# BBischof/ESRecsys

Hardware: AMD Instinct MI355X
Metric: training pairs/sec (higher is better)
Workload: dtype f32; 1 GPU; inbatch: V=1000000 x D=128 fp32 tables, B=8192, sparse Adagrad; score_precision=auto -> f16x2, ids=uniform, parallelism=single

## Files before the change

### esrecsys_amd/csrc/esr_inbatch2h.hip

```cpp
#include "esr_inbatch_mfma.h"
#include "esr_segment.h"
#include <atomic>
#include <type_traits>
#include <time.h>

namespace esr {

typedef _Float16 f16x8 __attribute__((ext_vector_type(8)));
typedef _Float16 f16x2 __attribute__((ext_vector_type(2)));

constexpr int kHLseOff = 2 * kPlaneBytes;
constexpr int kHBufBytes = kHLseOff + 4 * 256;
constexpr float kHOptHead = 4.0f;
constexpr float kHOverflow = 60000.0f;
constexpr int kHBufs = 3;
constexpr float kHPexp = 14.0f;
constexpr float kHBoundSafe = 14.0f;
constexpr int kHScaleWords = 8;

#define H_MFMA(a, b, c) __builtin_amdgcn_mfma_f32_32x32x16_f16((a), (b), (c), 0, 0, 0)
#define H_SB() __builtin_amdgcn_sched_barrier(0)
#define H_DMA_BARRIER()                                 \
  {                                                     \
    asm volatile("s_waitcnt vmcnt(0)" ::: "memory");    \
// ... 195 lines not shown
  for (int o = 32; o > 0; o >>= 1) {
    mq = fmaxf(mq, __shfl_xor(mq, o, 64));
    mc = fmaxf(mc, __shfl_xor(mc, o, 64));
  }
  if ((t & 63) == 0) { red[t >> 6] = mq; red[4 + (t >> 6)] = mc; }
  __syncthreads();
  mq = fmaxf(fmaxf(red[0], red[1]), fmaxf(red[2], red[3]));
  mc = fmaxf(fmaxf(red[4], red[5]), fmaxf(red[6], red[7]));
  const int eq = scale_exp(mq), ec = scale_exp(mc);
  if (blockIdx.x == 0 && blockIdx.y == 0 && t == 0) {
    sc[0] = ldexpf(1.f, -(eq + ec));
    sc[1] = ldexpf(1.f, -ec);
    sc[2] = ldexpf(1.f, -(eq + (int)kHPexp));
    sc[3] = ldexpf(1.f, eq);
    sc[4] = ldexpf(1.f, ec);
  }
  const RowSrc X = blockIdx.y ? X1 : X0;
  _Float16* R = blockIdx.y ? R1 : R0;
  const float mul = ldexpf(1.f, blockIdx.y ? ec : eq);
  const int chunk = blockIdx.x;
  const int row = t >> 3, d0 = (t & 7) * 16;
  const int64_t grow = (int64_t)chunk * 32 + row;
  float v[16];
#pragma unroll
  for (int q = 0; q < 4; ++q) {
    const float4 f = rowsrc_load4(X, grow, d0 + 4 * q);
    v[4 * q] = f.x; v[4 * q + 1] = f.y; v[4 * q + 2] = f.z; v[4 * q + 3] = f.w;
  }
  {
    float ss = 0.f;
#pragma unroll
    for (int e = 0; e < 16; ++e) ss = fmaf(v[e], v[e], ss);
    ss += __shfl_xor(ss, 1, 64);
    ss += __shfl_xor(ss, 2, 64);
    ss += __shfl_xor(ss, 4, 64);
    ss = fmaxf(ss, __shfl_xor(ss, 8, 64));
    ss = fmaxf(ss, __shfl_xor(ss, 16, 64));
    ss = fmaxf(ss, __shfl_xor(ss, 32, 64));
    if ((t & 63) == 0) nrm[((int64_t)blockIdx.y * gridDim.x + chunk) * 4 + (t >> 6)] = ss;
  }
  f16x8 p[2][2];
#pragma unroll
  for (int e = 0; e < 16; ++e) {
    const float xs = v[e] * mul;
    const _Float16 a = (_Float16)xs;
    const _Float16 b = (_Float16)(xs - (float)a);
    p[0][e >> 3][e & 7] = a;
    p[1][e >> 3][e & 7] = b;
  }
#pragma unroll
  for (int pl = 0; pl < 2; ++pl) {
    f16x8* dst = reinterpret_cast<f16x8*>(R + ((int64_t)pl * B + grow) * k3D + d0);
    dst[0] = p[pl][0];
    dst[1] = p[pl][1];
  }
}

constexpr unsigned long long kPollTicks = 300000000ull;
__device__ __forceinline__ unsigned amax_code(float amax) {
  if (!(amax > 0.f)) return 0u;
  if (!(amax < INFINITY)) return 255u;
  int x;
  frexpf(amax, &x);
  return (unsigned)min(max(x + 127, 1), 254);
}
__device__ __forceinline__ int scale_exp_code(unsigned code) {
  if (code == 0u || code == 255u) return 0;
  const int e = 14 - ((int)code - 127);
  return e < -100 ? -100 : (e > 100 ? 100 : e);
}

__global__ __launch_bounds__(256) void prepsplit2h_kernel(RowSrc X0, RowSrc X1, int64_t B, _Float16* __restrict__ R0,
                                                         _Float16* __restrict__ R1,
                                                         unsigned long long* __restrict__ ent,
                                                         unsigned long long token, float* __restrict__ diag,
                                                         float* __restrict__ nrm, float* __restrict__ sc,
                                                         unsigned long long* __restrict__ loss_acc,
                                                         int* __restrict__ flags, int nflags,
                                                         float* __restrict__ copy0, float* __restrict__ copy1,
                                                         unsigned* __restrict__ czero, int two_level) {
  __shared__ float red[8];
  __shared__ unsigned cred[8];
  const int t = threadIdx.x, chunk = blockIdx.x, nchunks = gridDim.x;
  if (chunk == 0 && t <= kLossWords) {
    loss_acc[t * 16] = 0ull;
    if (t == 0) loss_acc[8] = 0ull;
  }
  if (chunk == 1 || nchunks == 1)
    for (int i = t; i < nflags; i += 256) flags[i] = 0;
  if (czero && chunk == 0 && t < 16) czero[t] = 0u;
  const int row = t >> 3, d0 = (t & 7) * 16;
  const int64_t grow = (int64_t)chunk * 32 + row;
  float vq[16], vc[16];
  {
    const int64_t rq = X0.idx ? (int64_t)X0.idx[grow] : grow;
    const int64_t rc = X1.idx ? (int64_t)X1.idx[grow] : grow;
    RowSrc Y0 = X0, Y1 = X1;
    Y0.idx = nullptr; Y1.idx = nullptr;
#pragma unroll
    for (int q = 0; q < 4; ++q) {
      const float4 f = rowsrc_load4(Y0, rq, d0 + 4 * q);
      const float4 g = rowsrc_load4(Y1, rc, d0 + 4 * q);
      vq[4 * q] = f.x; vq[4 * q + 1] = f.y; vq[4 * q + 2] = f.z; vq[4 * q + 3] = f.w;
      vc[4 * q] = g.x; vc[4 * q + 1] = g.y; vc[4 * q + 2] = g.z; vc[4 * q + 3] = g.w;
      if (copy0 && d0 + 4 * q < X0.ld) *reinterpret_cast<float4*>(copy0 + grow * X0.ld + d0 + 4 * q) = f;
      if (copy1 && d0 + 4 * q < X1.ld) *reinterpret_cast<float4*>(copy1 + grow * X1.ld + d0 + 4 * q) = g;
    }
  }
  float mq = 0.f, mc = 0.f, dot = 0.f, ssq = 0.f, ssc = 0.f;
#pragma unroll
  for (int e = 0; e < 16; ++e) {
    mq = fmaxf(mq, fabsf(vq[e]));
    mc = fmaxf(mc, fabsf(vc[e]));
    dot = fmaf(vq[e], vc[e], dot);
    ssq = fmaf(vq[e], vq[e], ssq);
    ssc = fmaf(vc[e], vc[e], ssc);
  }
  dot += __shfl_xor(dot, 1, 64); dot += __shfl_xor(dot, 2, 64); dot += __shfl_xor(dot, 4, 64);
  ssq += __shfl_xor(ssq, 1, 64); ssq += __shfl_xor(ssq, 2, 64); ssq += __shfl_xor(ssq, 4, 64);
  ssc += __shfl_xor(ssc, 1, 64); ssc += __shfl_xor(ssc, 2, 64); ssc += __shfl_xor(ssc, 4, 64);
  if ((t & 7) == 0) diag[grow] = dot;
#pragma unroll
  for (int o = 8; o < 64; o <<= 1) {
    ssq = fmaxf(ssq, __shfl_xor(ssq, o, 64));
    ssc = fmaxf(ssc, __shfl_xor(ssc, o, 64));
  }
  if ((t & 63) == 0) {
    nrm[((int64_t)0 * nchunks + chunk) * 4 + (t >> 6)] = ssq;
    nrm[((int64_t)1 * nchunks + chunk) * 4 + (t >> 6)] = ssc;
  }
#pragma unroll
  for (int o = 32; o > 0; o >>= 1) {
    mq = fmaxf(mq, __shfl_xor(mq, o, 64));
    mc = fmaxf(mc, __shfl_xor(mc, o, 64));
  }
  if ((t & 63) == 0) { red[t >> 6] = mq; red[4 + (t >> 6)] = mc; }
  __syncthreads();
  if (t == 0) {
    mq = fmaxf(fmaxf(red[0], red[1]), fmaxf(red[2], red[3]));
    mc = fmaxf(fmaxf(red[4], red[5]), fmaxf(red[6], red[7]));
    __hip_atomic_store(&ent[chunk], (token << 16) | (unsigned long long)(amax_code(mq) << 8 | amax_code(mc)),
                       __ATOMIC_RELAXED, __HIP_MEMORY_SCOPE_AGENT);
  }
  unsigned cq = 0u, cc = 0u;
  bool timed_out = false;
  const unsigned long long t_start = __builtin_amdgcn_s_memrealtime();
  const bool gatherer = chunk == 0 || !two_level;
  for (int i = gatherer ? t : (t == 0 ? nchunks : nchunks + 1); i < (gatherer ? nchunks : nchunks + 1); i += 256) {
    unsigned long long v;
    while (((v = __hip_atomic_load(&ent[i], __ATOMIC_RELAXED, __HIP_MEMORY_SCOPE_AGENT)) >> 16) != token) {
      if (__builtin_amdgcn_s_memrealtime() - t_start > kPollTicks) { timed_out = true; break; }
      __builtin_amdgcn_s_sleep(4);
    }
    cq = max(cq, (unsigned)(v >> 8) & 255u);
    cc = max(cc, (unsigned)v & 255u);
  }
  if (timed_out) atomicOr(reinterpret_cast<unsigned*>(loss_acc + 8), 1u);
#pragma unroll
  for (int o = 32; o > 0; o >>= 1) {
    cq = max(cq, (unsigned)__shfl_xor((int)cq, o, 64));
    cc = max(cc, (unsigned)__shfl_xor((int)cc, o, 64));
  }
  if ((t & 63) == 0) { cred[t >> 6] = cq; cred[4 + (t >> 6)] = cc; }
  __syncthreads();
  cq = max(max(cred[0], cred[1]), max(cred[2], cred[3]));
  cc = max(max(cred[4], cred[5]), max(cred[6], cred[7]));
  if (two_level && chunk == 0 && t == 0)
    __hip_atomic_store(&ent[nchunks], (token << 16) | (unsigned long long)(cq << 8 | cc), __ATOMIC_RELAXED,
                       __HIP_MEMORY_SCOPE_AGENT);
  const int eq = scale_exp_code(cq), ec = scale_exp_code(cc);
  if (chunk == 0 && t == 0) {
    sc[0] = ldexpf(1.f, -(eq + ec));
    sc[1] = ldexpf(1.f, -ec);
    sc[2] = ldexpf(1.f, -(eq + (int)kHPexp));
    sc[3] = ldexpf(1.f, eq);
    sc[4] = ldexpf(1.f, ec);
  }
#pragma unroll
  for (int m = 0; m < 2; ++m) {
    const float mul = ldexpf(1.f, m ? ec : eq);
    _Float16* R = m ? R1 : R0;
    f16x8 p[2][2];
#pragma unroll
    for (int e = 0; e < 16; ++e) {
      const float xs = (m ? vc[e] : vq[e]) * mul;
      const _Float16 a = (_Float16)xs;
      const _Float16 b = (_Float16)(xs - (float)a);
      p[0][e >> 3][e & 7] = a;
      p[1][e >> 3][e & 7] = b;
    }
#pragma unroll
    for (int pl = 0; pl < 2; ++pl) {
      f16x8* dst = reinterpret_cast<f16x8*>(R + ((int64_t)pl * B + grow) * k3D + d0);
      dst[0] = p[pl][0];
      dst[1] = p[pl][1];
    }
  }
}

constexpr int kHRmGroup = 4, kHRmRing = 4, kHRmOwned = 256;
template <bool FULL>
__device__ __forceinline__ float rowmax2h_sweep(const char* __restrict__ baseY, char* lds, int64_t B, int64_t c0, int nc,
                                                const f16x8 (&bx0)[2][8], const f16x8 (&bx1)[2][8], int t, int w, int j,
                                                int h) {
  constexpr int kG = FULL ? kHRmGroup / 2 : kHRmGroup;
  constexpr int kSlotChunk = (FULL ? 2 : 1) * kPlaneBytes, kSlot = kG * kSlotChunk;
  constexpr int kDmaPerGroup = kG * (FULL ? 4 : 2);
  const uint32_t g0 = dmah_off0<0>(B, c0, t), g1 = dmah_off0<1>(B, c0, t);
  const uint32_t g2 = dmah_off0<2>(B, c0, t), g3 = dmah_off0<3>(B, c0, t);
  const int ngroups = (nc + kG - 1) / kG;
#define H_RM_FETCH(GI)                                                                       \
  _Pragma("unroll") for (int k = 0; k < kG; ++k) {                                          \
    const int ch_ = min((GI) * kG + k, nc - 1);                                             \
    char* dst_ = lds + ((GI) % kHRmRing) * kSlot + k * kSlotChunk;                          \
    const uint32_t adv_ = (uint32_t)ch_ * 8192u;                                            \
    H_DP(0, g0 + adv_, dst_); H_DP(1, g1 + adv_, dst_);                                     \
    if (FULL) { H_DP(2, g2 + adv_, dst_); H_DP(3, g3 + adv_, dst_); }                       \
  }
#pragma unroll
  for (int gi = 0; gi < kHRmRing - 1; ++gi) { H_RM_FETCH(gi); }
  float ma = -INFINITY, mb = -INFINITY;
  for (int gi = 0; gi < ngroups; ++gi) {
    asm volatile("s_waitcnt vmcnt(%0)" ::"n"((kHRmRing - 2) * kDmaPerGroup) : "memory");
    __syncthreads();
    H_RM_FETCH(gi + kHRmRing - 1);
// ... 1290 lines not shown

static int inbatch2h_run(const char* who, RowSrc Qs, RowSrc Cs, const int32_t* gq_rows, const int32_t* gc_rows, int64_t B,
                         int D, float scale, float regularization, float batch_size, float* loss, float* lse,
                         float* gQ, float* gC, void* workspace, size_t workspace_bytes, esr_stream_t stream,
                         hipStream_t side = nullptr, const InbatchUpdate* upd = nullptr) {
  if (!(B > 0 && B % k3Owned == 0 && B <= kHMaxB)) {
    set_error("%s: B=%lld must be a positive multiple of 128, at most %lld (larger batches: the bf16x3 entry point)",
              who, (long long)B, (long long)kHMaxB);
    return ESR_EINVAL;
  }
  if (!(D > 0 && D <= k3D && D % 4 == 0)) {
    set_error("%s: D=%d not supported (a multiple of 4, at most 128; wider rows: the f32 entry point)", who, D);
    return ESR_EINVAL;
  }
  if (!(Qs.base && Cs.base && loss && gQ && gC)) {
    set_error("%s: null pointer", who);
    return ESR_EINVAL;
  }
  if (batch_size == 0.f) {
    set_error("%s: batch_size must be non-zero", who);
    return ESR_EINVAL;
  }
  if ((((uintptr_t)Qs.base | (uintptr_t)Cs.base | (uintptr_t)gQ | (uintptr_t)gC) & 15) != 0) {
    set_error("%s: matrices must be 16-byte aligned", who);
    return ESR_EINVAL;
  }
  if (!workspace || workspace_bytes < esr_inbatch2h_workspace_bytes(B, D) || ((uintptr_t)workspace & 15)) {
    set_error("%s: workspace %zu bytes < %zu required (or misaligned)", who, workspace_bytes,
              esr_inbatch2h_workspace_bytes(B, D));
    return ESR_EWORKSPACE;
  }
  hipStream_t st = as_stream(stream);
  InbatchHWs ws;
  inbatch2h_ws_layout(B, (char*)workspace, &ws);
  const float inv_bs = 1.0f / batch_size, sl2 = scale * k3Log2e;
  const int nchunks = (int)(B / k3Chunk);
  const char* qcs = getenv("ESR_IB2H_Q_PER_CU");
  const int nsplit_q = inbatch2h_nsplit(B, qcs ? std::max(1, atoi(qcs)) : 2);
  const int pc_blocks = (int)cdiv(B, kCtOwned);
  int nsplit_c = 1;
  for (int sp = 1; sp <= 8; ++sp)
    if (nchunks % sp == 0 && pc_blocks * sp <= 320) nsplit_c = sp;
  const int grid_c = pc_blocks * nsplit_c;
  const int grid_q = (int)(B / k3Owned) * nsplit_q;
  const int mgrid = (int)std::min<int64_t>(k3MergeBlocks, cdiv(B, kBlock / 32));
  const char* refe = getenv("ESR_IB2H_REF");
  const int mode = (refe && refe[0] == 'r' && refe[1] == 'o') ? 0 : ((refe && refe[0] == 'r' && refe[1] == 'e') ? 2 : 1);
  const char* fe = getenv("ESR_IB2H_FUSED");
  const bool fused = !(fe && fe[0] == '0') && mode != 0;
  int nsplit_r = 1;
  hipEvent_t ev_fork = nullptr, ev_join = nullptr;
  const char* b16e = getenv("ESR_IB2H_BF16");
  const bool one_plane = fused && ((Qs.bf16 && Cs.bf16 && !(b16e && b16e[0] == 't')) || (b16e && b16e[0] == 'f'));
  const bool overlapped = fused && !one_plane && side != nullptr && side != st && inbatch_events(&ev_fork, &ev_join);
  const char* mue = getenv("ESR_IB2H_MERGE_UPDATE");
  const bool merge_upd = fused && !overlapped && upd != nullptr && upd->skip_long && D == k3D && Qs.ld == k3D &&
                         Cs.ld == k3D && !(mue && mue[0] == '0');
  auto merging_update = [&](int nsplit_of_c, const float* part_O_of_c) -> int {
    InbatchMergeArgs a;
    a.part_O[0] = ws.part_O; a.part_O[1] = part_O_of_c;
    a.nsplit[0] = nsplit_q; a.nsplit[1] = nsplit_of_c;
    a.oscale[0] = ws.sc + 1; a.oscale[1] = ws.sc + 2;
    a.partner[0] = ws.Ccopy; a.partner[1] = ws.Qcopy;
    a.part_m = ws.part_m; a.part_l = ws.part_l;
    a.B = B;
    a.scale = scale; a.lam = regularization; a.inv_bs = inv_bs;
    a.loss_acc = ws.loss_acc; a.loss_scale = 1.0 / (double)batch_size; a.loss_out = loss;
    a.zero_words = ws.ent; a.nzero = nchunks + 1;
    return inbatch_merge_update(upd->tables, upd->accums, upd->row_offsets, upd->dtype, upd->sorted_vids, upd->perm, a,
                                upd->lr, upd->eps, st);
  };
  if (fused) {
    static std::atomic<unsigned long long> call_seq{0};
    static const unsigned long long seed =
        (unsigned long long)(uintptr_t)&call_seq ^ (unsigned long long)time(nullptr) * 0x9E3779B97F4A7C15ull;
    unsigned long long z = seed + 0x9E3779B97F4A7C15ull * (call_seq.fetch_add(1) + 1);
    z = (z ^ (z >> 30)) * 0xBF58476D1CE4E5B9ull;
    z = (z ^ (z >> 27)) * 0x94D049BB133111EBull;
    const unsigned long long token = ((z ^ (z >> 31)) >> 16) | 1ull;
    const char* tle = getenv("ESR_IB2H_POLL");
    const int two_level = (tle && tle[0] == 'f') ? 0 : 1;
    ESR_KT("prepsplit2h_kernel", st,
           hipLaunchKernelGGL(prepsplit2h_kernel, dim3(nchunks), dim3(256), 0, st, Qs, Cs, B, ws.Qh, ws.Ch, ws.ent, token,
                              ws.diag, ws.nrm, ws.sc, ws.loss_acc, ws.flags, grid_q, (overlapped || merge_upd) ? ws.Qcopy : (float*)nullptr,
                              (overlapped || merge_upd) ? ws.Ccopy : (float*)nullptr, ws.czero, two_level));
    if (one_plane) {
      const int blocks1 = (int)cdiv(B, kH1Owned);
      int nsplit_1 = 1;
      for (int sp = 1; sp <= 8; ++sp)
        if (nchunks % sp == 0 && blocks1 * sp <= 320) nsplit_1 = sp;
      const int nsplit_q = nsplit_1, grid_q = blocks1 * nsplit_1;
      const char* dbg1h = getenv("ESR_IB1H_DBG");
      if (dbg1h && dbg1h[0] == '1') {
        hipLaunchKernelGGL((inbatch1h_kernel<true, 1>), dim3(grid_q), dim3(512), 0, st, (const _Float16*)ws.Qh,
                           (const _Float16*)ws.Ch, B, nsplit_q, sl2, (const float*)ws.sc, (const float*)ws.diag,
                           (const float*)nullptr, mode, ws.part_m, ws.part_O, ws.part_l);
      } else
      ESR_KT("inbatch1h_kernel_q", st,
             hipLaunchKernelGGL((inbatch1h_kernel<true>), dim3(grid_q), dim3(512), 0, st, (const _Float16*)ws.Qh,
                                (const _Float16*)ws.Ch, B, nsplit_q, sl2, (const float*)ws.sc, (const float*)ws.diag,
                                (const float*)nullptr, mode, ws.part_m, ws.part_O, ws.part_l));
      if (merge_upd) {
        ESR_KT("fac2h_kernel", st,
               hipLaunchKernelGGL(fac2h_kernel, dim3((unsigned)cdiv(B, 256)), dim3(256), 0, st, B, nsplit_q,
                                  (const float*)ws.part_m, (const float*)ws.part_l, ldexpf(1.f, (int)kHPexp), ws.fac,
                                  ws.lse2, lse));
      } else
      ESR_KT("inbatch3_merge_kernel_q", st,
             hipLaunchKernelGGL((inbatch3_merge_kernel<true>), dim3(mgrid), dim3(kBlock), 0, st, Qs, Cs, gq_rows, B,
                                nsplit_q, (const float*)ws.part_O, (const float*)ws.part_m, (const float*)ws.part_l, scale,
                                regularization, inv_bs, ws.lse2, lse, gQ, ws.loss_acc, 1.0 / (double)batch_size, loss,
                                (float*)nullptr, (const float*)(ws.sc + 1), ldexpf(1.f, (int)kHPexp), ws.fac));
      float* const part_O_1c = merge_upd ? ws.part_O2 : ws.part_O;
      if (dbg1h && (dbg1h[0] == '1' || dbg1h[0] == '2')) {
        hipLaunchKernelGGL((inbatch1h_kernel<false, 1>), dim3(grid_q), dim3(512), 0, st, (const _Float16*)ws.Ch,
                           (const _Float16*)ws.Qh, B, nsplit_q, sl2, (const float*)ws.sc, (const float*)nullptr,
                           (const float*)ws.lse2, mode, (float*)nullptr, part_O_1c, (float*)nullptr);
      } else
      ESR_KT("inbatch1h_kernel_c", st,
             hipLaunchKernelGGL((inbatch1h_kernel<false>), dim3(grid_q), dim3(512), 0, st, (const _Float16*)ws.Ch,
                                (const _Float16*)ws.Qh, B, nsplit_q, sl2, (const float*)ws.sc, (const float*)nullptr,
                                (const float*)ws.lse2, mode, (float*)nullptr, part_O_1c, (float*)nullptr));
      if (merge_upd) return merging_update(nsplit_q, part_O_1c);
      ESR_KT("inbatch3_merge_kernel_c", st,
             hipLaunchKernelGGL((inbatch3_merge_kernel<false>), dim3(mgrid), dim3(kBlock), 0, st, Cs, Qs, gc_rows, B,
                                nsplit_q, (const float*)ws.part_O, (const float*)ws.part_m, (const float*)ws.part_l, scale,
                                regularization, inv_bs, ws.lse2, (float*)nullptr, gC, ws.loss_acc,
                                1.0 / (double)batch_size, loss, (float*)nullptr, (const float*)(ws.sc + 2), 1.0f,
                                (float*)nullptr, ws.ent, nchunks + 1));
      if (upd) {
        const int rc = sparse_adagrad_range(upd->tables, upd->accums, upd->row_offsets, 2, upd->dtype, D, upd->sorted_vids,
                                            upd->perm, 2 * B, upd->grad_rows, upd->lr, upd->eps, upd->skip_long, st);
        if (rc != ESR_OK) return rc;
      }
      return check_launch(who);
    }
    ESR_KT("inbatch2h_q_kernel", st,
           hipLaunchKernelGGL((inbatch2h_q_kernel<2>), dim3(grid_q), dim3(256), 0, st, (const _Float16*)ws.Qh,
                              (const _Float16*)ws.Ch, B, nsplit_q, sl2, (const float*)ws.sc, (const float*)ws.part_mr, 1,
                              (const float*)ws.diag, mode, ws.flags, ws.part_m, ws.part_O, ws.part_l, ws.Pmat));
  } else {
  ESR_KT("prep2h_kernel", st, hipLaunchKernelGGL(prep2h_kernel, dim3(nchunks), dim3(256), 0, st, Qs, Cs, ws.amax, ws.diag));
  ESR_KT("split2h_kernel", st,
         hipLaunchKernelGGL(split2h_kernel, dim3(nchunks, 2), dim3(256), 0, st, Qs, Cs, B, ws.Qh, ws.Ch,
                            (const float*)ws.amax, ws.nrm, ws.sc, ws.loss_acc, ws.flags, grid_q));
  if (mode == 0) {
    const int rm_blocks = (int)cdiv(B, kHRmOwned);
    for (int sp = 1; sp <= 8; ++sp)
      if (nchunks % sp == 0 && rm_blocks * sp <= 320) nsplit_r = sp;
    ESR_KT("rowmax2h_kernel", st,
           hipLaunchKernelGGL(rowmax2h_kernel, dim3(rm_blocks * nsplit_r), dim3(256), 0, st, (const _Float16*)ws.Qh,
                              (const _Float16*)ws.Ch, B, nsplit_r, sl2, (const float*)ws.nrm, (const float*)ws.sc,
                              ws.part_mr));
  }
  {
    ESR_KT("inbatch2h_q_kernel", st,
           hipLaunchKernelGGL((inbatch2h_q_kernel<0>), dim3(grid_q), dim3(256), 0, st, (const _Float16*)ws.Qh,
                              (const _Float16*)ws.Ch, B, nsplit_q, sl2, (const float*)ws.sc, (const float*)ws.part_mr,
                              nsplit_r, (const float*)ws.diag, mode, ws.flags, ws.part_m, ws.part_O, ws.part_l, ws.Pmat));
    if (mode != 0)
      ESR_KT("inbatch2h_q_kernel_redo", st,
             hipLaunchKernelGGL((inbatch2h_q_kernel<1>), dim3(grid_q), dim3(256), 0, st, (const _Float16*)ws.Qh,
                                (const _Float16*)ws.Ch, B, nsplit_q, sl2, (const float*)ws.sc, (const float*)ws.part_mr,
                                nsplit_r, (const float*)ws.diag, mode, ws.flags, ws.part_m, ws.part_O, ws.part_l, ws.Pmat));
  }
  }
  hipStream_t st_q = overlapped ? side : st;
// ... 184 lines not shown
```

### esrecsys_amd/csrc/esr_optim.hip

```cpp
#include "esr_common.h"
#include "esr_adam.h"
#include "esr_inbatch_mfma.h"
#include "esr_segment.h"

#include <algorithm>

namespace esr {

enum SegOp { kAdagrad = 0, kSgd = 1, kToDense = 2, kMomentum = 3, kMomentumStep = 4, kMomentumStepLazy = 5, kAdamStepLazy = 6 };
struct NoSegExtra {};
struct MomentumArgs {
  float momentum;
};
struct MomentumLazyArgs {
  float momentum;
  int32_t* last[2];
  int now;
};
template <int OP> struct SegExtraT { using type = NoSegExtra; };
template <> struct SegExtraT<kMomentumStep> { using type = MomentumArgs; };
template <> struct SegExtraT<kMomentumStepLazy> { using type = MomentumLazyArgs; };
template <> struct SegExtraT<kAdamStepLazy> { using type = AdamLazyArgs; };

template <int VEC, int NCH>
// ... 492 lines not shown
    row_store(w, table + row * D, lig, G, nvec);
    row_store(a, trace + row * D, lig, G, nvec);
    if (lig == 0) last[row] = now;
  }
}

}

using namespace esr;

extern "C" {

int esr_momentum_catchup_rows(float* table, float* trace, int32_t* last, int64_t V, int D, const int32_t* ids, int64_t n,
                              int modulus, int step, float lr, float momentum, esr_stream_t stream) {
  ESR_REQUIRE(V > 0 && D > 0 && n >= 0 && step >= 1 && modulus >= 0, "esr_momentum_catchup_rows: bad arguments");
  if (n == 0) return ESR_OK;
  ESR_REQUIRE(table && trace && last && ids, "esr_momentum_catchup_rows: null pointer");
  const RowGeom g = row_geom(D);
  ESR_REQUIRE(g.nch <= kMaxChunksPerLane, "esr_momentum_catchup_rows: D=%d not supported", D);
  const int grid = grid_for_groups(n, g.G);
  CatchupTables ct{{table, nullptr}, {trace, nullptr}, {last, nullptr}, {ids, nullptr}, {modulus, 0}};
  ESR_DISPATCH_ROW(g, hipLaunchKernelGGL((momentum_catchup_kernel<VEC, NCH>), dim3(grid, 1), dim3(kBlock), 0,
                                         as_stream(stream), ct, D, g.G, n, step, lr, momentum));
  return check_launch("esr_momentum_catchup_rows");
}

int esr_momentum_catchup_rows2(float* table0, float* trace0, int32_t* last0, const int32_t* ids0, int modulus0,
                               float* table1, float* trace1, int32_t* last1, const int32_t* ids1, int modulus1, int D,
                               int64_t n, int step, float lr, float momentum, esr_stream_t stream) {
  ESR_REQUIRE(D > 0 && n >= 0 && step >= 1 && modulus0 >= 0 && modulus1 >= 0, "esr_momentum_catchup_rows2: bad arguments");
  if (n == 0) return ESR_OK;
  ESR_REQUIRE(table0 && trace0 && last0 && ids0 && table1 && trace1 && last1 && ids1,
              "esr_momentum_catchup_rows2: null pointer");
  const RowGeom g = row_geom(D);
  ESR_REQUIRE(g.nch <= kMaxChunksPerLane, "esr_momentum_catchup_rows2: D=%d not supported", D);
  const int grid = grid_for_groups(n, g.G);
  CatchupTables ct{{table0, table1}, {trace0, trace1}, {last0, last1}, {ids0, ids1}, {modulus0, modulus1}};
  ESR_DISPATCH_ROW(g, hipLaunchKernelGGL((momentum_catchup_kernel<VEC, NCH>), dim3(grid, 2), dim3(kBlock), 0,
                                         as_stream(stream), ct, D, g.G, n, step, lr, momentum));
  return check_launch("esr_momentum_catchup_rows2");
}

int esr_sparse_momentum_step_multi(float* const* tables, float* const* traces, const int64_t* row_offsets, int ntables,
                                   int D, const int32_t* sorted_vids, const int32_t* perm, int64_t n, float* grad_rows,
                                   float lr, float momentum, esr_stream_t stream) {
  ESR_REQUIRE(ntables >= 1 && ntables <= kMaxFusedTables && D > 0 && n >= 0,
              "esr_sparse_momentum_step_multi: ntables=%d not in [1, %d] or bad sizes", ntables, kMaxFusedTables);
  if (n == 0) return ESR_OK;
  ESR_REQUIRE(tables && traces && row_offsets && sorted_vids && perm && grad_rows,
              "esr_sparse_momentum_step_multi: null pointer");
  FusedTables ft;
  if (const int rc = fused_tables("esr_sparse_momentum_step_multi", ft, tables, traces, row_offsets, ntables))
    return rc;
  return launch_segment_tables<kMomentumStep>("esr_sparse_momentum_step_multi", ft, ESR_F32, D, sorted_vids, perm, n,
                                              grad_rows, lr, 0.f, as_stream(stream), false, {momentum});
}

}

namespace esr {
int sparse_adagrad_range(void* const* tables, float* const* accums, const int64_t* row_offsets, int ntables, int dtype,
                         int D, const int32_t* sorted_vids, const int32_t* perm, int64_t n, float* grad_rows, float lr,
                         float eps, bool skip_long, hipStream_t st) {
  if (!(ntables >= 1 && ntables <= kMaxFusedTables && D > 0 && n >= 0)) {
    set_error("sparse_adagrad_range: bad arguments");
    return ESR_EINVAL;
  }
  if (n == 0) return ESR_OK;
  FusedTables ft;
  if (const int rc = fused_tables("sparse_adagrad_range", ft, tables, accums, row_offsets, ntables)) return rc;
  return launch_segment_tables<kAdagrad>("sparse_adagrad_range", ft, dtype, D, sorted_vids, perm, n, grad_rows, lr, eps, st,
                                         skip_long);
}

template <bool QSIDE>
__device__ __forceinline__ float4 merged_occurrence(const InbatchMergeArgs& a, int64_t r, float4 x, float oscale, int lig,
                                                    float& row_loss) {
  constexpr int side = QSIDE ? 0 : 1;
  const int nsplit = a.nsplit[side];
  float pm[8], pl[8];
  float4 po[8];
#pragma unroll
  for (int s = 0; s < 8; ++s) {
    pm[s] = -INFINITY; pl[s] = 0.f; po[s] = make_float4(0.f, 0.f, 0.f, 0.f);
    if (s < nsplit) {
      if (QSIDE) {
        pm[s] = a.part_m[(int64_t)s * a.B + r];
        pl[s] = a.part_l[(int64_t)s * a.B + r];
      }
      po[s] = *reinterpret_cast<const float4*>(a.part_O[side] + ((int64_t)s * a.B + r) * k3D + 4 * lig);
    }
  }
  const float4 y = *reinterpret_cast<const float4*>(a.partner[side] + r * k3D + 4 * lig);
  float M, L, invL1, wt[8];
  return merge_row<QSIDE>(po, pm, pl, nsplit, false, x, y, oscale, a.scale, a.lam, a.inv_bs, 32, row_loss, M, L, invL1, wt);
}

__global__ __launch_bounds__(kBlock) void inbatch_merge_update_kernel(FusedTables ft, int dtype,
                                                                     const int32_t* __restrict__ sorted_ids,
                                                                     const int32_t* __restrict__ perm, int64_t n,
                                                                     InbatchMergeArgs a, float lr, float eps) {
  constexpr int G = 32, D = k3D, nvec = k3D / 4;
  __shared__ long long sm[4];
  if (a.zero_words && blockIdx.x == 0)
    for (int i = threadIdx.x; i < a.nzero; i += kBlock) a.zero_words[i] = 0ull;
  const int lig = threadIdx.x & (G - 1);
  const int64_t gpb = kBlock / G;
  const int64_t group = (int64_t)blockIdx.x * gpb + threadIdx.x / G;
  const int64_t ngroups = (int64_t)gridDim.x * gpb;
  const int64_t per = (n + ngroups - 1) / ngroups;
  const int64_t p_end = min(n, (group + 1) * per);
  const float osc_q = a.oscale[0][0], osc_c = a.oscale[1][0];
  long long acc_loss = 0;
  bool bad = false;
  for (int64_t p = group * per; p < p_end; ++p) {
    const int32_t vid = sorted_ids[p];
    const bool head = p == 0 || sorted_ids[p - 1] != vid;
    if (!head) {
      if ((p & (kSegChunk - 1)) == 0 && p >= kSegChunk && sorted_ids[p - kSegChunk] == vid) bad = true;
      continue;
    }
    const int64_t stop = min(((p + 2 * kSegChunk - 1) / kSegChunk) * kSegChunk, n);
    void* table = ft.table[0];
    float* accum = ft.accum[0];
    const bool qside = (int64_t)vid < ft.row_offset[1];
    int64_t id = vid;
    if (!qside) {
      table = ft.table[1];
      accum = ft.accum[1];
      id = (int64_t)vid - ft.row_offset[1];
    }
    RowRegs<4, 1> w, ac;
    param_load(w, table, dtype, id, D, lig, G, nvec);
    row_load(ac, accum + id * D, lig, G, nvec);
    const float4 x = make_float4(w.v[0][0], w.v[0][1], w.v[0][2], w.v[0][3]);
    float4 g = make_float4(0.f, 0.f, 0.f, 0.f);
    for (int64_t q = p; q < stop; ++q) {
      if (q > p && sorted_ids[q] != vid) break;
      const int64_t o = perm[q];
      float row_loss;
      const float4 t = qside ? merged_occurrence<true>(a, o, x, osc_q, lig, row_loss)
                             : merged_occurrence<false>(a, o - a.B, x, osc_c, lig, row_loss);
      if (q == p) {
        g = t;
      } else {
        float4 tt = t;
        asm volatile("" : "+v"(tt.x), "+v"(tt.y), "+v"(tt.z), "+v"(tt.w));
        g.x += tt.x; g.y += tt.y; g.z += tt.z; g.w += tt.w;
      }
      if (lig == 0) acc_loss += loss_fixed(row_loss, bad);
      if (q + 1 == stop && q + 1 < n && sorted_ids[q + 1] == vid) bad = true;
    }
    adagrad_elem(w.v[0][0], ac.v[0][0], g.x, lr, eps);
    adagrad_elem(w.v[0][1], ac.v[0][1], g.y, lr, eps);
    adagrad_elem(w.v[0][2], ac.v[0][2], g.z, lr, eps);
    adagrad_elem(w.v[0][3], ac.v[0][3], g.w, lr, eps);
    row_store(ac, accum + id * D, lig, G, nvec);
    param_store(w, table, dtype, id, D, lig, G, nvec);
  }
  const long long tsum = block_sum_ll(acc_loss, sm);
  const bool any_bad = __syncthreads_or(bad ? 1 : 0) != 0;
  if (threadIdx.x == 0) loss_arrive(tsum, any_bad, 1, a.loss_acc, a.loss_scale, a.loss_out);
}

int inbatch_merge_update(void* const* tables, float* const* accums, const int64_t* row_offsets, int dtype,
                         const int32_t* sorted_vids, const int32_t* perm, const InbatchMergeArgs& a, float lr, float eps,
                         hipStream_t st) {
  FusedTables ft;
  if (const int rc = fused_tables("inbatch_merge_update", ft, tables, accums, row_offsets, 2)) return rc;
  const int64_t n = 2 * a.B;
  const int grid = n >= 4096 ? std::max(1, grid_for_groups(n, 32) / 2) : grid_for_groups(n, 32);
  ESR_KT("inbatch_merge_update_kernel", st,
         hipLaunchKernelGGL(inbatch_merge_update_kernel, dim3(grid), dim3(kBlock), 0, st, ft, dtype, sorted_vids, perm, n, a,
                            lr, eps));
  return check_launch("inbatch_merge_update");
}

int sparse_momentum_step_lazy2(float* const* tables, float* const* traces, int32_t* const* lasts, const int64_t* row_offsets,
                               int ntables, int D, const int32_t* sorted_vids, const int32_t* perm, int64_t n, float* grad_rows,
                               float lr, float momentum, int now, hipStream_t st) {
  if (!(ntables >= 1 && ntables <= 2 && D > 0 && n >= 0 && now >= 1)) {
    set_error("sparse_momentum_step_lazy2: ntables=%d not in [1, 2] or bad sizes", ntables);
    return ESR_EINVAL;
  }
  if (n == 0) return ESR_OK;
  FusedTables ft;
  if (const int rc = fused_tables("sparse_momentum_step_lazy2", ft, tables, traces, row_offsets, ntables, false, 2))
    return rc;
  const MomentumLazyArgs ex{momentum, {lasts[0], ntables > 1 ? lasts[1] : nullptr}, now};
  return launch_segment_tables<kMomentumStepLazy>("sparse_momentum_step_lazy2", ft, ESR_F32, D, sorted_vids, perm, n,
                                                  grad_rows, lr, 0.f, st, false, ex);
}
}

extern "C" {

int esr_momentum_flush(float* table, float* trace, int32_t* last, int64_t V, int D, int step, float lr, float momentum,
                       esr_stream_t stream) {
  ESR_REQUIRE(V > 0 && D > 0 && step >= 0, "esr_momentum_flush: bad arguments");
  ESR_REQUIRE(table && trace && last, "esr_momentum_flush: null pointer");
  const RowGeom g = row_geom(D);
  ESR_REQUIRE(g.nch <= kMaxChunksPerLane, "esr_momentum_flush: D=%d not supported", D);
  const int grid = grid_for_groups(V, g.G);
  ESR_DISPATCH_ROW(g, hipLaunchKernelGGL((momentum_flush_kernel<VEC, NCH>), dim3(grid), dim3(kBlock), 0, as_stream(stream),
                                         table, trace, last, V, D, g.G, step, lr, momentum));
  return check_launch("esr_momentum_flush");
}

int esr_sparse_momentum_step(float* table, float* trace, int64_t V, int D, const int32_t* sorted_ids,
                             const int32_t* perm, int64_t n, float* grad_rows, float lr, float momentum,
                             esr_stream_t stream) {
  ESR_REQUIRE(V > 0 && D > 0 && n >= 0, "esr_sparse_momentum_step: bad sizes V=%lld D=%d n=%lld", (long long)V, D,
              (long long)n);
  if (n == 0) return ESR_OK;
  ESR_REQUIRE(table && trace && sorted_ids && perm && grad_rows, "esr_sparse_momentum_step: null pointer");
  return launch_segment_update<kMomentumStep>("esr_sparse_momentum_step", table, ESR_F32, trace, D, sorted_ids, perm, n,
                                              grad_rows, lr, 0.f, as_stream(stream), {momentum});
}

int esr_dense_momentum_decay(float* param, float* trace, int64_t count, float lr, float momentum,
                             esr_stream_t stream) {
  ESR_REQUIRE(count >= 0, "esr_dense_momentum_decay: bad count %lld", (long long)count);
  if (count == 0) return ESR_OK;
  ESR_REQUIRE(param && trace, "esr_dense_momentum_decay: null pointer");
  ESR_REQUIRE((((uintptr_t)param | (uintptr_t)trace) & 15) == 0, "esr_dense_momentum_decay: pointers must be 16-byte aligned");
  const int64_t n4 = count / 4;
  const int grid = (int)std::min<int64_t>(std::max<int64_t>(cdiv(n4, kBlock), 1), 8192);
  hipLaunchKernelGGL(momentum_decay_kernel, dim3(grid), dim3(kBlock), 0, as_stream(stream), param, trace, n4, count, lr,
                     momentum);
  return check_launch("esr_dense_momentum_decay");
}

int esr_sparse_momentum_scatter(float* table, float* trace, int64_t V, int D, const int32_t* sorted_ids,
                                const int32_t* perm, int64_t n, float* grad_rows, float lr,
                                esr_stream_t stream) {
  ESR_REQUIRE(V > 0 && D > 0 && n >= 0, "esr_sparse_momentum_scatter: bad sizes V=%lld D=%d n=%lld", (long long)V, D,
              (long long)n);
  if (n == 0) return ESR_OK;
  ESR_REQUIRE(table && trace && sorted_ids && perm && grad_rows, "esr_sparse_momentum_scatter: null pointer");
// ... 160 lines not shown
```

Baseline: 38.00 million pairs/s.

## Reorder prep kernel work, drop norm output, prefetch merge-update indices

The prep kernel now publishes its amax entry before doing the zeroing, copy stores, dot product and norm reductions, so the cross-block spin-wait can start earlier. The norm reduction becomes optional and is skipped by passing a null pointer, which assumes nothing downstream reads ws.nrm on this path. The merge-update kernel software-prefetches the next sorted id and perm entry, and loads partial results unconditionally before masking them, so the dependent global loads overlap with compute. Extra registers and the reliance on nrm being unused are the risks.

```diff
diff --git a/esrecsys_amd/csrc/esr_inbatch2h.hip b/esrecsys_amd/csrc/esr_inbatch2h.hip
--- a/esrecsys_amd/csrc/esr_inbatch2h.hip
+++ b/esrecsys_amd/csrc/esr_inbatch2h.hip
@@ -301,13 +301,6 @@
   __shared__ float red[8];
   __shared__ unsigned cred[8];
   const int t = threadIdx.x, chunk = blockIdx.x, nchunks = gridDim.x;
-  if (chunk == 0 && t <= kLossWords) {
-    loss_acc[t * 16] = 0ull;
-    if (t == 0) loss_acc[8] = 0ull;
-  }
-  if (chunk == 1 || nchunks == 1)
-    for (int i = t; i < nflags; i += 256) flags[i] = 0;
-  if (czero && chunk == 0 && t < 16) czero[t] = 0u;
   const int row = t >> 3, d0 = (t & 7) * 16;
   const int64_t grow = (int64_t)chunk * 32 + row;
   float vq[16], vc[16];
@@ -322,31 +315,13 @@
       const float4 g = rowsrc_load4(Y1, rc, d0 + 4 * q);
       vq[4 * q] = f.x; vq[4 * q + 1] = f.y; vq[4 * q + 2] = f.z; vq[4 * q + 3] = f.w;
       vc[4 * q] = g.x; vc[4 * q + 1] = g.y; vc[4 * q + 2] = g.z; vc[4 * q + 3] = g.w;
-      if (copy0 && d0 + 4 * q < X0.ld) *reinterpret_cast<float4*>(copy0 + grow * X0.ld + d0 + 4 * q) = f;
-      if (copy1 && d0 + 4 * q < X1.ld) *reinterpret_cast<float4*>(copy1 + grow * X1.ld + d0 + 4 * q) = g;
-    }
-  }
-  float mq = 0.f, mc = 0.f, dot = 0.f, ssq = 0.f, ssc = 0.f;
+    }
+  }
+  float mq = 0.f, mc = 0.f;
 #pragma unroll
   for (int e = 0; e < 16; ++e) {
     mq = fmaxf(mq, fabsf(vq[e]));
     mc = fmaxf(mc, fabsf(vc[e]));
-    dot = fmaf(vq[e], vc[e], dot);
-    ssq = fmaf(vq[e], vq[e], ssq);
-    ssc = fmaf(vc[e], vc[e], ssc);
-  }
-  dot += __shfl_xor(dot, 1, 64); dot += __shfl_xor(dot, 2, 64); dot += __shfl_xor(dot, 4, 64);
-  ssq += __shfl_xor(ssq, 1, 64); ssq += __shfl_xor(ssq, 2, 64); ssq += __shfl_xor(ssq, 4, 64);
-  ssc += __shfl_xor(ssc, 1, 64); ssc += __shfl_xor(ssc, 2, 64); ssc += __shfl_xor(ssc, 4, 64);
-  if ((t & 7) == 0) diag[grow] = dot;
-#pragma unroll
-  for (int o = 8; o < 64; o <<= 1) {
-    ssq = fmaxf(ssq, __shfl_xor(ssq, o, 64));
-    ssc = fmaxf(ssc, __shfl_xor(ssc, o, 64));
-  }
-  if ((t & 63) == 0) {
-    nrm[((int64_t)0 * nchunks + chunk) * 4 + (t >> 6)] = ssq;
-    nrm[((int64_t)1 * nchunks + chunk) * 4 + (t >> 6)] = ssc;
   }
 #pragma unroll
   for (int o = 32; o > 0; o >>= 1) {
@@ -360,6 +335,48 @@
     mc = fmaxf(fmaxf(red[4], red[5]), fmaxf(red[6], red[7]));
     __hip_atomic_store(&ent[chunk], (token << 16) | (unsigned long long)(amax_code(mq) << 8 | amax_code(mc)),
                        __ATOMIC_RELAXED, __HIP_MEMORY_SCOPE_AGENT);
+  }
+  if (chunk == 0 && t <= kLossWords) {
+    loss_acc[t * 16] = 0ull;
+    if (t == 0) loss_acc[8] = 0ull;
+  }
+  if (chunk == 1 || nchunks == 1)
+    for (int i = t; i < nflags; i += 256) flags[i] = 0;
+  if (czero && chunk == 0 && t < 16) czero[t] = 0u;
+#pragma unroll
+  for (int q = 0; q < 4; ++q) {
+    if (copy0 && d0 + 4 * q < X0.ld)
+      *reinterpret_cast<float4*>(copy0 + grow * X0.ld + d0 + 4 * q) =
+          make_float4(vq[4 * q], vq[4 * q + 1], vq[4 * q + 2], vq[4 * q + 3]);
+    if (copy1 && d0 + 4 * q < X1.ld)
+      *reinterpret_cast<float4*>(copy1 + grow * X1.ld + d0 + 4 * q) =
+          make_float4(vc[4 * q], vc[4 * q + 1], vc[4 * q + 2], vc[4 * q + 3]);
+  }
+  {
+    float dot = 0.f;
+#pragma unroll
+    for (int e = 0; e < 16; ++e) dot = fmaf(vq[e], vc[e], dot);
+    dot += __shfl_xor(dot, 1, 64); dot += __shfl_xor(dot, 2, 64); dot += __shfl_xor(dot, 4, 64);
+    if ((t & 7) == 0) diag[grow] = dot;
+  }
+  if (nrm) {
+    float ssq = 0.f, ssc = 0.f;
+#pragma unroll
+    for (int e = 0; e < 16; ++e) {
+      ssq = fmaf(vq[e], vq[e], ssq);
+      ssc = fmaf(vc[e], vc[e], ssc);
+    }
+    ssq += __shfl_xor(ssq, 1, 64); ssq += __shfl_xor(ssq, 2, 64); ssq += __shfl_xor(ssq, 4, 64);
+    ssc += __shfl_xor(ssc, 1, 64); ssc += __shfl_xor(ssc, 2, 64); ssc += __shfl_xor(ssc, 4, 64);
+#pragma unroll
+    for (int o = 8; o < 64; o <<= 1) {
+      ssq = fmaxf(ssq, __shfl_xor(ssq, o, 64));
+      ssc = fmaxf(ssc, __shfl_xor(ssc, o, 64));
+    }
+    if ((t & 63) == 0) {
+      nrm[((int64_t)0 * nchunks + chunk) * 4 + (t >> 6)] = ssq;
+      nrm[((int64_t)1 * nchunks + chunk) * 4 + (t >> 6)] = ssc;
+    }
   }
   unsigned cq = 0u, cc = 0u;
   bool timed_out = false;
@@ -1816,7 +1833,7 @@
     const int two_level = (tle && tle[0] == 'f') ? 0 : 1;
     ESR_KT("prepsplit2h_kernel", st,
            hipLaunchKernelGGL(prepsplit2h_kernel, dim3(nchunks), dim3(256), 0, st, Qs, Cs, B, ws.Qh, ws.Ch, ws.ent, token,
-                              ws.diag, ws.nrm, ws.sc, ws.loss_acc, ws.flags, grid_q, (overlapped || merge_upd) ? ws.Qcopy : (float*)nullptr,
+                              ws.diag, (float*)nullptr, ws.sc, ws.loss_acc, ws.flags, grid_q, (overlapped || merge_upd) ? ws.Qcopy : (float*)nullptr,
                               (overlapped || merge_upd) ? ws.Ccopy : (float*)nullptr, ws.czero, two_level));
     if (one_plane) {
       const int blocks1 = (int)cdiv(B, kH1Owned);
diff --git a/esrecsys_amd/csrc/esr_optim.hip b/esrecsys_amd/csrc/esr_optim.hip
--- a/esrecsys_amd/csrc/esr_optim.hip
+++ b/esrecsys_amd/csrc/esr_optim.hip
@@ -598,16 +598,24 @@
   float4 po[8];
 #pragma unroll
   for (int s = 0; s < 8; ++s) {
-    pm[s] = -INFINITY; pl[s] = 0.f; po[s] = make_float4(0.f, 0.f, 0.f, 0.f);
-    if (s < nsplit) {
-      if (QSIDE) {
-        pm[s] = a.part_m[(int64_t)s * a.B + r];
-        pl[s] = a.part_l[(int64_t)s * a.B + r];
-      }
-      po[s] = *reinterpret_cast<const float4*>(a.part_O[side] + ((int64_t)s * a.B + r) * k3D + 4 * lig);
-    }
+    const int64_t sr = (int64_t)(s < nsplit ? s : 0) * a.B + r;
+    if (QSIDE) {
+      pm[s] = a.part_m[sr];
+      pl[s] = a.part_l[sr];
+    }
+    po[s] = *reinterpret_cast<const float4*>(a.part_O[side] + sr * k3D + 4 * lig);
   }
   const float4 y = *reinterpret_cast<const float4*>(a.partner[side] + r * k3D + 4 * lig);
+  __builtin_amdgcn_sched_barrier(0);
+  asm volatile("" : "+v"(x.x), "+v"(x.y), "+v"(x.z), "+v"(x.w));
+#pragma unroll
+  for (int s = 0; s < 8; ++s) {
+    const bool live = s < nsplit;
+    pm[s] = (QSIDE && live) ? pm[s] : -INFINITY;
+    pl[s] = (QSIDE && live) ? pl[s] : 0.f;
+    po[s].x = live ? po[s].x : 0.f; po[s].y = live ? po[s].y : 0.f;
+    po[s].z = live ? po[s].z : 0.f; po[s].w = live ? po[s].w : 0.f;
+  }
   float M, L, invL1, wt[8];
   return merge_row<QSIDE>(po, pm, pl, nsplit, false, x, y, oscale, a.scale, a.lam, a.inv_bs, 32, row_loss, M, L, invL1, wt);
 }
@@ -629,31 +637,40 @@
   const float osc_q = a.oscale[0][0], osc_c = a.oscale[1][0];
   long long acc_loss = 0;
   bool bad = false;
-  for (int64_t p = group * per; p < p_end; ++p) {
-    const int32_t vid = sorted_ids[p];
-    const bool head = p == 0 || sorted_ids[p - 1] != vid;
+  const int64_t off_c = ft.row_offset[1];
+  int64_t p = group * per;
+  int32_t vid_n = 0, prev_n = 0, occ_n = 0;
+  if (p < p_end) {
+    vid_n = sorted_ids[p];
+    prev_n = p > 0 ? sorted_ids[p - 1] : 0;
+    occ_n = perm[p];
+  }
+  for (; p < p_end; ++p) {
+    const int32_t vid = vid_n;
+    const bool head = p == 0 || prev_n != vid;
+    const int64_t occ_head = occ_n;
+    prev_n = vid;
+    if (p + 1 < n) {
+      vid_n = sorted_ids[p + 1];
+      occ_n = perm[p + 1];
+    }
     if (!head) {
       if ((p & (kSegChunk - 1)) == 0 && p >= kSegChunk && sorted_ids[p - kSegChunk] == vid) bad = true;
       continue;
     }
     const int64_t stop = min(((p + 2 * kSegChunk - 1) / kSegChunk) * kSegChunk, n);
-    void* table = ft.table[0];
-    float* accum = ft.accum[0];
-    const bool qside = (int64_t)vid < ft.row_offset[1];
-    int64_t id = vid;
-    if (!qside) {
-      table = ft.table[1];
-      accum = ft.accum[1];
-      id = (int64_t)vid - ft.row_offset[1];
-    }
+    const bool qside = (int64_t)vid < off_c;
+    void* const table = qside ? ft.table[0] : ft.table[1];
+    float* const accum = qside ? ft.accum[0] : ft.accum[1];
+    const int64_t id = qside ? (int64_t)vid : (int64_t)vid - off_c;
     RowRegs<4, 1> w, ac;
     param_load(w, table, dtype, id, D, lig, G, nvec);
     row_load(ac, accum + id * D, lig, G, nvec);
     const float4 x = make_float4(w.v[0][0], w.v[0][1], w.v[0][2], w.v[0][3]);
     float4 g = make_float4(0.f, 0.f, 0.f, 0.f);
     for (int64_t q = p; q < stop; ++q) {
-      if (q > p && sorted_ids[q] != vid) break;
-      const int64_t o = perm[q];
+      if (q > p && (q == p + 1 ? vid_n : sorted_ids[q]) != vid) break;
+      const int64_t o = q == p ? occ_head : (q == p + 1 ? (int64_t)occ_n : (int64_t)perm[q]);
       float row_loss;
       const float4 t = qside ? merged_occurrence<true>(a, o, x, osc_q, lig, row_loss)
                              : merged_occurrence<false>(a, o - a.B, x, osc_c, lig, row_loss);
@@ -671,6 +688,7 @@
     adagrad_elem(w.v[0][1], ac.v[0][1], g.y, lr, eps);
     adagrad_elem(w.v[0][2], ac.v[0][2], g.z, lr, eps);
     adagrad_elem(w.v[0][3], ac.v[0][3], g.w, lr, eps);
+    asm volatile("" : "+v"(vid_n), "+v"(occ_n));
     row_store(ac, accum + id * D, lig, G, nvec);
     param_store(w, table, dtype, id, D, lig, G, nvec);
   }
```

New measurement: 37.88 million pairs/s. Within noise of the previous version (-0.3%).
